# weleen/AGRL.pytorch

Measured on AMD Instinct MI355X. Metric: frames/sec (fwd+GCN+distmat), MARS seq_len=8, higher is better.
Workload: dtype fp16; 1 GPU; MARS seq_len=8 bs=32/GPU fp16 fwd+distmat (BASELINE configs[1]): 256x128 frames, VMGN ResNet50x2-branch + 2 graph layers, cosine distmat vs resident 12180 x 4096 gallery; global_batch=32, seq_len=8, gallery_rows_per_gpu=12180, parallelism=dp1, hip_graph=False, ranks=1, devices_visible=1, library=libagrl_hip.so, clip_batches_rotated=3, clip_bytes_rotated=301989888

## Files before the change

agrl.pytorch_amd/torchreid/_hip.py:

```python
from __future__ import annotations

import ctypes as C
import os
import threading

import torch

F32 = 0
LP16 = 1
F32X3 = 2
F32H3P = 4
F32H3 = 3
FRAMES_NCHW = 0
FRAMES_NHWC = 1
METRIC_EUCLIDEAN = 0
METRIC_COSINE = 1

LP_NAME = os.environ.get("AGRL_HIP_LP16")
if LP_NAME is None:
    LP_NAME = os.environ.get("AGRL_HIP_PRECISION") if os.environ.get("AGRL_HIP_PRECISION") in ("fp16", "bf16") else "fp16"
if LP_NAME not in ("fp16", "bf16"):
    raise ValueError("AGRL_HIP_LP16 must be fp16 or bf16, not %r" % LP_NAME)
LP_DTYPE = torch.float16 if LP_NAME == "fp16" else torch.bfloat16

_HERE = os.path.dirname(os.path.abspath(__file__))
LIB_PATH = os.environ.get(
    "AGRL_HIP_LIB", os.path.normpath(os.path.join(_HERE, "..", "lib", "libagrl_hip.so" if LP_NAME == "fp16" else "libagrl_hip_bf16.so"))
)


class HipLibraryError(RuntimeError):
    """libagrl_hip.so is missing or incomplete."""


class HipKernelError(RuntimeError):
    """An entry point of libagrl_hip.so returned a non-zero status."""


_p = C.c_void_p
_i = C.c_int
_f = C.c_float

SIGNATURES = {
    "agrl_stem_conv_bn_relu_maxpool": [_p, _p, _p, _p, _i, _i, _i, _i, _p],
    "agrl_stem_conv_bn_relu_maxpool_lp16": [_p, _p, _p, _p, _i, _i, _i, _p],
    "agrl_conv2d_bn_act": [_p, _p, _p, _p, _p, _i, _i, _i, _i, _i, _i, _i, _i, _i, _i, _i, _p],
    "agrl_conv1x1_dual_split16": [_p, _p, _p, _p, _p] + [_i] * 8 + [_f, _i, _i, _p],
    "agrl_stem_split16": [_p, _p, _p, _p, _p, _i, _i, _i, _f, _p],
    "agrl_stem_conv_bn_relu_maxpool_u8": [_p, _p, _i, _p, _p, _p, _i, _i, _i, _i, _p],
    "agrl_stem_conv_bn_relu_maxpool_lp16_u8": [_p, _p, _i, _p, _p, _p, _i, _i, _i, _p],
    "agrl_stem_split16_u8": [_p, _p, _i, _p, _p, _p, _p, _i, _i, _i, _f, _p],
    "agrl_frames_normalize_u8": [_p, _p, _i, _p, _i, _i, _i, _p],
    "agrl_split16_planes": [_p, _p, C.c_longlong, _i, _i, _p],
    "agrl_split16_weight_planes": [_p, _p, C.c_longlong, _i, _f, _p],
    "agrl_split16_weights_inloop": [_p, _p, C.c_longlong, _i, _p],
    "agrl_conv1x1_split16": [_p, _p, _p, _p, _p, _i, _i, _i, _i, _f, _i, _p],
    "agrl_conv1x1_split16_dual": [_p, _p, _p, _p, _p, _i, _i, _i, _i, _i, _f, _i, _p],
    "agrl_conv1x1_split16_pool": [_p, _p, _p, _p, _p, _i, _i, _i, _i, _i, _i, C.POINTER(_i), _i, _i, _f, _i, _p],
    "agrl_conv3x3_packed_split16": [_p, _p, _p, _p, _i, _i, _i, _i, _i, _i, _f, _p],
    "agrl_conv2d_bn_act_split16": [_p, _p, _p, _p, _p] + [_i] * 10 + [_f, _i, _i, _p],
    "agrl_bottleneck_tail": [_p, _p, _p, _p, _p, _p, _p, _p, _p, _p, _p, _i, _i, _i, _i, _i, _p],
    "agrl_bottleneck_seam_packed_bytes": [_i, _i, _i],
    "agrl_bottleneck_seam_pack": [_p, _p, _p, _i, _i, _i, _p],
    "agrl_bottleneck_seam": [_p, _p, _p, _p, _p, _p, _p, _i, _i, _i, _i, _p],
    "agrl_conv3x3_packed_bytes": [_i, _i],
    "agrl_conv1x1_packed_bytes": [_i, _i],
    "agrl_conv1x1_pack": [_p, _p, _i, _i, _p],
    "agrl_conv1x1_packed_bn_act": [_p, _p, _p, _p, _p, _i, _i, _i, _i, _i, _p],
    "agrl_conv1x1_packed_res_bn_act": [_p, _p, _p, _p, _p, _i, _i, _i, _i, _p],
    "agrl_conv1x1_packed_res_pool": [_p, _p, _p, _p, _p, _p, _i, _i, _i, _i, _i, _i, C.POINTER(_i), _i, _i, _p],
    "agrl_conv1x1_packed_dual_duo": [_p, _p, _p, _p, _p, _i, _i, _i, _i, _i, _p],
    "agrl_conv1x1_packed_dual_strided": [_p, _p, _p, _p, _p, _i, _i, _i, _i, _i, _i, _i, _i, _p],
    "agrl_conv3x3_pack": [_p, _p, _i, _i, _p],
    "agrl_conv3x3_packed_bn_act": [_p, _p, _p, _p, _i, _i, _i, _i, _i, _i, _p],
    "agrl_bottleneck_block": [_p, _p, _p, _p, _p, _p, _p, _p, _p, _p, _p, _p, _p, _i, _i, _i, _i, _i, _i, _p],
    "agrl_conv1x1_dual_bn_act": [_p, _p, _p, _p, _p, _i, _i, _i, _i, _i, _p],
    "agrl_conv1x1_bn_act_pool": [_p, _p, _p, _p, _p, _p, _p, _i, _i, _i, _i, _i, _i, C.POINTER(_i), _i, _i, _p],
    "agrl_linear_nobias": [_p, _p, _p, _i, _i, _i, _i, _p],
    "agrl_part_pool": [_p, _p, _p, _p, _p, _i, _i, _i, _i, C.POINTER(_i), _i, _i, _p],
    "agrl_clip_pool": [_p, _p, _i, _i, _i, _i, _p],
    "agrl_graph_gram": [_p, _p, _i, _i, _i, _i, _p],
    "agrl_graph_pair_product": [_p, _p, _p, _p, _i, _i, _i, _p],
    "agrl_graph_finalize": [_p, _i, _p, _p, _i, _i, _i, _i, _i, _p],
    "agrl_graph_propagate": [_p, _p, _p, _p, _p, _f, _f, _f, _p, _p, _i, _i, _i, _p],
    "agrl_pam_pool": [_p, _p, _p, _p, _i, _i, _i, _i, _i, C.POINTER(_i), _i, _i, _p],
    "agrl_pam_combine": [_p, _p, _p, _f, _p, _p, _i, _i, _p],
    "agrl_graph_apply": [_p, _p, _p, _i, _i, _i, _i, _p],
    "agrl_graph_tracklet_operand": [_p, _p, _i, _p, _p, _i, _i, _i, _i, _i, _i, _i, _p],
    "agrl_graph_finalize_bits": [_p, _i, _p, _p, _i, _i, _i, _i, _i, _p],
    "agrl_pose_adjacency_bits": [_p, _p, _p, _i, _i, _i, _i, C.c_float, C.c_float, _p],
    "agrl_adjacency_pack": [_p, _p, _i, _i, _p],
    "agrl_graph_linear_mix": [_p, _p, _p, _p, _p, _f, _f, _f, _p, _i, _i, _i, _i, _p],
    "agrl_row_sqnorm": [_p, _p, _i, _i, _i, _p],
    "agrl_attn_pool_bnneck": [_p, _p, _p, _p, _p, _p, _p, _p, _p, _p, _i, _i, _i, _i, _i, _p],
    "agrl_attn_tail": [_p, _p, _p, _p, _p, _p, _p, _p, _p, _p, _p, _p, _p, _i, _i, _i, _i, _i, _p],
    "agrl_row_l2_normalize": [_p, _p, _i, _i, _i, _i, _i, _p],
    "agrl_distmat_split16": [_p, _p, _p, _p, _p, _i, _i, _i, _i, _i, _f, _p, C.c_size_t, _p],
    "agrl_distmat": [_p, _p, _p, _p, _p, _i, _i, _i, _i, _i, _i, _p, C.c_size_t, _p],
    "agrl_pose_adjacency": [_p, _p, _p, _i, _i, _i, _i, C.c_float, C.c_float, _p],
    "agrl_re_ranking_workspace": [_i, _i, _i],
    "agrl_re_ranking": [_p, _p, _p, _i, _i, _i, _i, C.c_double, _p, _i, _p, C.c_size_t, _p],
    "agrl_rank_topk": [_p, _i, _i, _i, _i, _i, _p, _p, _p],
    "agrl_distmat_topk_workspace": [_i, _i],
    "agrl_distmat_topk": [_p, _p, _p, _p, _i, _i, _i, _i, _i, _i, _i, _p, _p, _p, C.c_size_t, _p, C.c_size_t, _p],
    "agrl_rank_argsort": [_p, _i, _i, _i, _p, _p],
    "agrl_rank_mars": [_p, _p, _p, _p, _p, _i, _i, _i, _p, _p, _p],
    "agrl_rank_market1501": [_p, _i, _i, _i, _p, _p, _p, _p, _i, _p, _p, _p, _p],
    "agrl_triplet_hard_mine": [_p, _p, _i, _i, _p, _p, _p, _p, _p],
    "agrl_axpby": [_p, _p, _f, _f, _p, C.c_size_t, _p],
    "agrl_part_pool_backward": [_p, _p, _p, _p, _i, _i, _i, _i, _i, C.POINTER(_i), _i, _p],
    "agrl_attn_pool_backward": [_p, _p, _p, _i, _i, _i, _i, _p],
    "agrl_graph_matrix_backward": [_p, _i, _p, _p, _i, _i, _i, _i, _p],
    "agrl_xent_label_smooth": [_p, _p, _i, _i, _f, _p, _p, _p, _p],
    "agrl_triplet_loss": [_p, _p, _i, _i, _f, _i, _p, _p, _p, _p, _p, _p, _p, _p],
    "agrl_bn_workspace": [_i, _i],
    "agrl_bn_stats": [_p, _p, _p, _i, _i, _p, C.c_size_t, _p],
    "agrl_conv2d_stats": [_p, _p, _p, _p, C.c_size_t] + [_i] * 10 + [_p],
    "agrl_bn_stats_from_partials": [_p, _i, _i, _i, _p, _p, _p, C.c_size_t, _p],
    "agrl_bn_fold_train": [_p, _p, _p, _p, _f, _f, C.c_longlong, _p, _p, _p, _p, _p, _p, _i, _p],
    "agrl_bn_apply": [_p, _p, _p, _p, _p, _p, _i, _i, _i, _f, _p],
    "agrl_bn_backward": [_p, _p, _p, _p, _p, _p, _p, _i, _f, _p, _p, _p, _p, _i, _i, _p, C.c_size_t, _p],
    "agrl_im2col_t": [_p, _p, _i, _i, _i, _i, _i, _i, _i, _i, _i, _p],
    "agrl_gemm_nt_splitk": [_p, _p, _p, _i, _i, _i, _i, _p, C.c_size_t, _p],
    "agrl_im2col_rows": [_p, _p] + [_i] * 10 + [_p],
    "agrl_conv_wgrad_workspace": [_i] * 9,
    "agrl_conv_wgrad_plan": [_i] * 10 + [C.POINTER(_i)],
    "agrl_conv_wgrad": [_p, _p, _p] + [_i] * 10 + [_p, C.c_size_t, _p],
    "agrl_maxpool3x3s2": [_p, _p, _p, _i, _i, _i, _i, _p],
    "agrl_maxpool3x3s2_backward": [_p, _p, _p, _i, _i, _i, _i, _p],
    "agrl_diag_read_stream": [_p, C.c_size_t, _p, _i, _p],
    "agrl_optim_geometry": [C.POINTER(_i), C.POINTER(_i), C.POINTER(_i)],
    "agrl_adam_step": [_p, _i, _p, _i] + [_f] * 7 + [_i, _i, _p],
    "agrl_sgd_step": [_p, _i, _p, _i, _f, _f, _f, _i, _i, _i, _i, _p],
}

_lock = threading.Lock()
_lib = None


def lib():
    global _lib
    if _lib is not None:
        return _lib
    with _lock:
        if _lib is not None:
            return _lib
        if not os.path.exists(LIB_PATH):
            raise HipLibraryError(
                "libagrl_hip.so not found at %s -- build it with `python __graft_entry__.py` "
                "(or `make -C agrl.pytorch_amd/csrc`); the HIP path has no fallback" % LIB_PATH
            )
        try:
            h = C.CDLL(LIB_PATH)
        except OSError as e:
            raise HipLibraryError("cannot load %s: %s" % (LIB_PATH, e))
        for name, argtypes in SIGNATURES.items():
            try:
                fn = getattr(h, name)
            except AttributeError:
                raise HipLibraryError("%s does not export %s" % (LIB_PATH, name))
            fn.argtypes = argtypes
            fn.restype = _i
        h.agrl_re_ranking_workspace.restype = C.c_size_t
        h.agrl_bn_workspace.restype = C.c_size_t
        h.agrl_conv_wgrad_workspace.restype = C.c_size_t
        h.agrl_distmat_topk_workspace.restype = C.c_size_t
        h.agrl_bottleneck_seam_packed_bytes.restype = C.c_longlong
        h.agrl_conv3x3_packed_bytes.restype = C.c_longlong
        h.agrl_conv1x1_packed_bytes.restype = C.c_longlong
        for name in ("agrl_reload_options", "agrl_built_with_ablation", "agrl_lp16_is_f16"):
            getattr(h, name).argtypes = []
            getattr(h, name).restype = _i
        h.agrl_version.restype = _i
        h.agrl_last_error.restype = C.c_char_p
        if bool(h.agrl_lp16_is_f16()) != (LP_NAME == "fp16"):
            raise HipLibraryError("%s stores 16-bit data as %s but AGRL_HIP_LP16 asks for %s" % (
                LIB_PATH, "fp16" if h.agrl_lp16_is_f16() else "bf16", LP_NAME))
        _lib = h
    return _lib


RELOAD_HOOKS = []


def reload_options():
    lib().agrl_reload_options()
    for hook in RELOAD_HOOKS:
        hook()


def available() -> bool:
    try:
        lib()
        return True
    except HipLibraryError:
        return False


def _check(name, status):
    if status != 0:
        msg = lib().agrl_last_error()
        raise HipKernelError("%s failed (%d): %s" % (name, status, msg.decode() if msg else "?"))


def stream_ptr(device=None):
    return torch.cuda.current_stream(device).cuda_stream


def ptr(t):
    if t is None:
        return None
    assert t.is_cuda, "HIP entry points take device tensors"
    assert t.is_contiguous(), "HIP entry points take contiguous tensors"
    return t.data_ptr()


def dtype_code(dt):
    if dt == torch.float32:
        return F32
    if dt == LP_DTYPE:
        return LP16
    raise TypeError("unsupported dtype %s (float32 / %s only: the loaded library's 16-bit type is %s)" % (dt, LP_DTYPE, LP_NAME))


PROFILE = None
PROFILE_TAG = None


def call(name, *args):
    fn = getattr(lib(), name)
    if PROFILE is None:
        _check(name, fn(*args))
        return
    stream = torch.cuda.ExternalStream(args[-1]) if args[-1] else torch.cuda.current_stream()
    start, end = torch.cuda.Event(enable_timing=True), torch.cuda.Event(enable_timing=True)
    start.record(stream)
    _check(name, fn(*args))
    end.record(stream)
    global PROFILE_TAG
    PROFILE.append((name, start, end, PROFILE_TAG))
    PROFILE_TAG = None
```

agrl.pytorch_amd/torchreid/hip_ops.py:

```python
from __future__ import annotations

import ctypes as C
import os

import torch

from . import _hip
from ._hip import F32, LP16, LP_DTYPE, LP_NAME, METRIC_COSINE, METRIC_EUCLIDEAN, call, dtype_code, ptr


import contextlib
import threading
import weakref

_MODE = threading.local()


@contextlib.contextmanager
def f32_split(on=True):
    prev = getattr(_MODE, 'split', False)
    _MODE.split = bool(on)
    try:
        yield
    finally:
# ... 458 lines not shown


def bottleneck_seam(y2, packed, b3, residual, b1_next, dims):
    Cmid, Cout, Cnext = dims
    N, H, W, C = y2.shape
    M = N * H * W
    assert y2.dtype == LP_DTYPE and C == Cmid and residual.shape == (N, H, W, Cout) and residual.dtype == y2.dtype and M % 128 == 0
    assert y2.is_contiguous() and residual.is_contiguous()
    out = torch.empty((N, H, W, Cout), dtype=y2.dtype, device=y2.device)
    z = torch.empty((N, H, W, Cnext), dtype=y2.dtype, device=y2.device)
    if _hip.PROFILE is not None:
        _hip.PROFILE_TAG = {"flops": 2.0 * M * (Cmid * Cout + Cout * Cnext),
                            "bytes": 2.0 * (y2.numel() + residual.numel() + out.numel() + z.numel()) + packed.numel(),
                            "conv": (1, 1, Cmid, Cout, H, W)}
    with _dev(y2):
        call("agrl_bottleneck_seam", ptr(y2), ptr(packed), ptr(b3), ptr(residual), ptr(out), ptr(b1_next), ptr(z), M, Cmid, Cout,
             Cnext, _stream(y2))
    return out, z


def conv3x3_packed_enabled():
    return True


def conv3x3_packed_supported(w_ohwi, H=None, W=None):
    return (w_ohwi.dtype == LP_DTYPE and w_ohwi.dim() == 4 and tuple(w_ohwi.shape[1:3]) == (3, 3) and w_ohwi.shape[3] % 64 == 0
            and w_ohwi.shape[3] >= 128 and (w_ohwi.shape[0] % 256 == 0 or w_ohwi.shape[0] == 128) and (H is None or (H % 16 == 0 and W % 8 == 0)))


def conv3x3_pack(w_ohwi):
    assert conv3x3_packed_supported(w_ohwi)
    Cout, Cin = w_ohwi.shape[0], w_ohwi.shape[3]
    if Cout == 128:
        w_ohwi = torch.cat([w_ohwi, torch.zeros_like(w_ohwi)], dim=0)
        Cout = 256
    w_ohwi = w_ohwi.contiguous()
    nbytes = int(_hip.lib().agrl_conv3x3_packed_bytes(Cin, Cout))
    assert nbytes == 2 * w_ohwi.numel()
    packed = torch.empty((nbytes,), dtype=torch.uint8, device=w_ohwi.device)
    with _dev(w_ohwi):
        call("agrl_conv3x3_pack", ptr(w_ohwi), ptr(packed), Cin, Cout, _stream(w_ohwi))
    return packed


def conv3x3_packed(x, packed, bias, Cout, relu=True):
    N, H, W, Cin = x.shape
    assert x.dtype == LP_DTYPE and x.is_contiguous() and packed.numel() == 2 * 9 * Cin * max(Cout, 256)
    out = torch.empty((N, H, W, Cout), dtype=x.dtype, device=x.device)
    if _hip.PROFILE is not None:
        _hip.PROFILE_TAG = {"flops": 2.0 * N * H * W * 9 * Cin * Cout, "bytes": 2.0 * (x.numel() + out.numel()) + 2.0 * 9 * Cin * Cout,
                            "conv": (3, 1, Cin, Cout, H, W)}
    with _dev(x):
        call("agrl_conv3x3_packed_bn_act", ptr(x), ptr(packed), ptr(bias), ptr(out), N, H, W, Cin, Cout, 1 if relu else 0, _stream(x))
    return out


def conv1x1_packed_supported(w):
    w2 = w.reshape(w.shape[0], -1) if w.dim() == 4 and tuple(w.shape[1:3]) == (1, 1) else w
    return w2.dtype == LP_DTYPE and w2.dim() == 2 and w2.shape[1] % 128 == 0 and w2.shape[0] % 256 == 0


def conv1x1_pack(w):
    assert conv1x1_packed_supported(w)
    w = w.reshape(w.shape[0], -1).contiguous()
    Cout, K = w.shape
    nbytes = int(_hip.lib().agrl_conv1x1_packed_bytes(K, Cout))
    assert nbytes == 2 * w.numel()
    packed = torch.empty((nbytes,), dtype=torch.uint8, device=w.device)
    with _dev(w):
        call("agrl_conv1x1_pack", ptr(w), ptr(packed), K, Cout, _stream(w))
    return packed


def conv1x1_packed(x, packed, bias, Cout, relu=True, x2=None, duo=False):
    N, H, W, K1 = x.shape
    K2 = 0 if x2 is None else x2.shape[3]
    M = N * H * W
    assert x.dtype == LP_DTYPE and x.is_contiguous() and packed.numel() == 2 * (K1 + K2) * Cout
    assert x2 is None or (x2.dtype == x.dtype and x2.is_contiguous() and tuple(x2.shape[:3]) == (N, H, W))
    out = torch.empty((N, H, W, Cout), dtype=x.dtype, device=x.device)
    if _hip.PROFILE is not None:
        _hip.PROFILE_TAG = {"flops": 2.0 * M * (K1 + K2) * Cout,
                            "bytes": 2.0 * (x.numel() + (0 if x2 is None else x2.numel()) + out.numel()) + packed.numel(),
                            "conv": (1, 1, K1 + K2, Cout, H, W)}
    with _dev(x):
        if duo and x2 is not None:
            call("agrl_conv1x1_packed_dual_duo", ptr(x), ptr(x2), ptr(packed), ptr(bias), ptr(out), M, K1, K2, Cout, 1 if relu else 0, _stream(x))
        else:
            call("agrl_conv1x1_packed_bn_act", ptr(x), ptr(x2), ptr(packed), ptr(bias), ptr(out), M, K1, K2, Cout, 1 if relu else 0, _stream(x))
    return out


def conv1x1_packed_dual_strided(x, x2, packed, bias, Cout, stride, relu=True):
    N, Hi, Wi, K1 = x.shape
    Ho, Wo = (Hi - 1) // stride + 1, (Wi - 1) // stride + 1
    K2 = x2.shape[3]
    assert x.dtype == LP_DTYPE and x2.dtype == LP_DTYPE and x.is_contiguous() and x2.is_contiguous()
    assert tuple(x2.shape[:3]) == (N, Ho, Wo) and packed.numel() == 2 * (K1 + K2) * Cout
    out = torch.empty((N, Ho, Wo, Cout), dtype=x.dtype, device=x.device)
    M = N * Ho * Wo
    if _hip.PROFILE is not None:
        _hip.PROFILE_TAG = {"flops": 2.0 * M * (K1 + K2) * Cout, "bytes": 2.0 * (M * K1 + x2.numel() + out.numel()) + packed.numel(),
                            "conv": (1, 1, K1 + K2, Cout, Ho, Wo)}
    with _dev(x):
        call("agrl_conv1x1_packed_dual_strided", ptr(x), ptr(x2), ptr(packed), ptr(bias), ptr(out), N, Hi, Wi, stride, K1, K2, Cout,
             1 if relu else 0, _stream(x))
# ... 812 lines not shown
```

agrl.pytorch_amd/torchreid/models/_vmgn_hip.py:

```python
from __future__ import annotations

import os

import torch

from torchreid import hip_ops as ops
from torchreid import _hip

_PRECISIONS = {'fp32': torch.float32, ops.LP_NAME: ops.LP_DTYPE, 'bf16x3': torch.float32, 'fp16x3': torch.float32}


def _fold_conv_bn(conv, bn, dtype, split16=False):
    w = conv.weight.detach().float()
    scale = bn.weight.detach().float() / torch.sqrt(bn.running_var.detach().float() + bn.eps)
    shift = bn.bias.detach().float() - bn.running_mean.detach().float() * scale
    w = (w * scale.view(-1, 1, 1, 1)).permute(0, 2, 3, 1).contiguous()
    if split16:
        assert dtype == torch.float32
        return ops.split16_inloop_weights(w), shift.contiguous()
    return w.to(dtype).contiguous(), shift.contiguous()


def check_packed_range(pack, where="vmgn"):
    def walk(obj, path):
# ... 5 lines not shown
            for k, v in obj.items():
                walk(v, "%s.%s" % (path, k))
        elif isinstance(obj, (list, tuple)):
            for i, v in enumerate(obj):
                walk(v, "%s[%d]" % (path, i))
    walk({k: v for k, v in pack.items() if k != 'fingerprint'}, "pack")


def _fold_bn1d(bn):
    scale = bn.weight.detach().float() / torch.sqrt(bn.running_var.detach().float() + bn.eps)
    shift = bn.bias.detach().float() - bn.running_mean.detach().float() * scale
    return scale.contiguous(), shift.contiguous()


def _pack_stage(stage, dtype, seam=False, split16=False):
    blocks = []
    for unit in stage:
        blk = {
            'c1': _fold_conv_bn(unit.conv1, unit.bn1, dtype, split16),
            'c2': _fold_conv_bn(unit.conv2, unit.bn2, dtype, split16),
            'c3': _fold_conv_bn(unit.conv3, unit.bn3, dtype, split16),
            'stride': unit.conv2.stride[0],
            'ds': None,
        }
        if unit.downsample is not None:
            blk['ds'] = _fold_conv_bn(unit.downsample[0], unit.downsample[1], dtype, split16)
            blk['ds_stride'] = unit.downsample[0].stride[0]
            if split16 and blk['ds_stride'] == blk['stride'] and blk['ds'][0].shape[3] % 32 == 0 and blk['c3'][0].shape[3] % 32 == 0:
                cout = blk['c3'][0].shape[0]
                wd = ops.split16_true_weights(blk['ds'][0])
                w3 = ops.split16_true_weights(blk['c3'][0])
                blk['dual16'] = (ops.split16_inloop_weights(torch.cat([wd.view(cout, -1), w3.view(cout, -1)], dim=1).contiguous()),
                                 (blk['ds'][1] + blk['c3'][1]).contiguous())
            if dtype == ops.LP_DTYPE and blk['ds_stride'] == 1 and blk['stride'] == 1:
                cout = blk['c3'][0].shape[0]
                blk['dual'] = (torch.cat([blk['ds'][0].view(cout, -1), blk['c3'][0].view(cout, -1)], dim=1).contiguous(),
                               (blk['ds'][1] + blk['c3'][1]).contiguous())
                if (ops.conv1x1_packed_supported(blk['dual'][0]) and blk['dual'][0].shape[1] >= 1536
                        and blk['ds'][0].shape[3] % 128 == 0 and blk['c3'][0].shape[3] % 128 == 0):
                    blk['dualp'] = ops.conv1x1_pack(blk['dual'][0])
            if dtype == ops.LP_DTYPE and blk['ds_stride'] > 1 and blk['ds_stride'] == blk['stride']:
                cout = blk['c3'][0].shape[0]
                dual_w = torch.cat([blk['ds'][0].view(cout, -1), blk['c3'][0].view(cout, -1)], dim=1).contiguous()
                if (ops.conv1x1_packed_supported(dual_w) and blk['ds'][0].shape[3] % 128 == 0 and blk['c3'][0].shape[3] % 128 == 0):
                    blk['dualps'] = ops.conv1x1_pack(dual_w)
                    blk['dualps_bias'] = (blk['ds'][1] + blk['c3'][1]).contiguous()
        if dtype == ops.LP_DTYPE and ops.conv1x1_packed_supported(blk['c1'][0]) and blk['c1'][0].shape[3] >= 1024:
            blk['c1p'] = ops.conv1x1_pack(blk['c1'][0])
        if (dtype == ops.LP_DTYPE and blk['ds'] is None and ops.conv1x1_packed_supported(blk['c3'][0])
                and blk['c3'][0].shape[0] >= 2048):
            blk['c3p'] = ops.conv1x1_pack(blk['c3'][0])
        if dtype == ops.LP_DTYPE and blk['stride'] == 1 and ops.conv3x3_packed_supported(blk['c2'][0]):
            blk['c2p'] = ops.conv3x3_pack(blk['c2'][0])
        blocks.append(blk)
    if seam and dtype == ops.LP_DTYPE:
        for blk, nxt in zip(blocks[:-1], blocks[1:]):
            if ops.bottleneck_seam_supported(blk['c3'][0], nxt['c1'][0]):
                blk['seam'] = ops.bottleneck_seam_pack(blk['c3'][0], nxt['c1'][0])
                blk['seam_dims'] = (blk['c3'][0].shape[3], blk['c3'][0].shape[0], nxt['c1'][0].shape[0])
    return blocks


def K_OK(w):
    return w.dim() == 2 and w.shape[1] % 32 == 0


def _fingerprint(model):
    return tuple((t.data_ptr(), t._version) for t in list(model.parameters()) + list(model.buffers()))


def pack_weights(model, device, precision):
    ops.check_precision(precision)
    key = (device.index if device.index is not None else torch.cuda.current_device(), precision)
    cached = model._hip_packs.get(key)
    if cached is not None and (model.hip_static_weights or cached['fingerprint'] == _fingerprint(model)):
        return cached
    first = next(model.parameters())
    if first.device != device:
        raise RuntimeError('model parameters live on {} but the input is on {}'.format(first.device, device))
    dtype = _PRECISIONS[precision]
    s16 = precision == 'fp16x3'
    with torch.no_grad():
        stem_w, stem_b = _fold_conv_bn(model.conv1, model.bn1, torch.float32)
        pack = {
            'dtype': dtype,
            'stem': (stem_w, stem_b),
            'stem_lp': ops.pack_stem_weights_lp16(stem_w) if dtype == ops.LP_DTYPE else None,
            'stem_s16': ops.pack_stem_weights_split16(stem_w) if s16 else None,
            'trunk': _pack_stage(model.layer1, dtype, split16=s16) + _pack_stage(model.layer2, dtype, split16=s16) + _pack_stage(model.layer3, dtype, seam=True, split16=s16),
            'graph': [],
        }
        if hasattr(model, 'layer4_1'):
            pack['l4_1'] = _pack_stage(model.layer4_1, dtype, split16=s16)
            pack['l4_2'] = _pack_stage(model.layer4_2, dtype, split16=s16)
            pack['g_bn'] = _fold_bn1d(model.global_bottleneck)
            pack['a_bn'] = _fold_bn1d(model.att_bottleneck)
        else:
            pack['l4'] = _pack_stage(model.layer4, dtype, split16=s16)
            pack['a_bn'] = _fold_bn1d(model.bottleneck)
            pack['g_bn'] = (torch.ones_like(pack['a_bn'][0]), torch.zeros_like(pack['a_bn'][1]))
        for layer in model.graph_layers:
            scale, shift = _fold_bn1d(layer.bn)
            gw = layer.linear.weight.detach().to(dtype).contiguous()
            if s16 and K_OK(gw):
                gw = ops.split16_inloop_weights(gw)
                scale = (scale * gw.agrl_unscale).contiguous()
# ... 24 lines not shown
        check_packed_range(pack)
    pack['fingerprint'] = _fingerprint(model)
    model._hip_packs[key] = pack
    return pack


def _pack_planes(blk):
    def true_w(pair):
        return ops.split16_true_weights(pair[0])

    w1, w2, w3 = true_w(blk['c1']), true_w(blk['c2']), true_w(blk['c3'])
    K1, K3c, mid, cout = w1.shape[3], w3.shape[3], w1.shape[0], w3.shape[0]
    if blk['stride'] != 1 or mid % 256 or cout % 256 or K1 % 128 or K3c % 128 or tuple(w2.shape[1:3]) != (3, 3) or w2.shape[3] % 64:
        return False
    p3 = {}
    t, u = ops.split16_plane_weights(w1.view(mid, K1), pair_first=True)
    p3['c1'] = (ops.conv1x1_pack(t), u, blk['c1'][1], mid)
    t, u = ops.split16_plane_weights(w2)
    p3['c2'] = (ops.conv3x3_pack(t), u, blk['c2'][1], w2.shape[0])
    if blk['ds'] is not None:
        if blk['ds_stride'] != 1:
            return False
        wd = true_w(blk['ds'])
        Kd = wd.shape[3]
        if Kd % 128:
            return False
        t, u = ops.split16_plane_weights(torch.cat([wd.view(cout, Kd), w3.view(cout, K3c)], dim=1), segments=[Kd, K3c], pair_first=True)
        p3['dual'] = (ops.conv1x1_pack(t), u, (blk['ds'][1] + blk['c3'][1]).contiguous(), cout)
    else:
        t, u = ops.split16_plane_weights(w3.view(cout, K3c))
        p3['c3'] = (ops.conv1x1_pack(t), u, blk['c3'][1], cout)
    blk['p3'] = p3
    return True


def _run_block_planes(x3, blk, pool=None):
    p3 = blk['p3']
    xp, rop = 1, 2
    y = ops.conv1x1_split16(x3, p3['c1'][0], p3['c1'][1], p3['c1'][2], p3['c1'][3], layout=xp)
    y = ops.conv3x3_split16(y, p3['c2'][0], p3['c2'][1], p3['c2'][2], p3['c2'][3])
    if 'dual' in p3:
        assert pool is None
        d = p3['dual']
        return ops.conv1x1_split16(x3, d[0], d[1], d[2], d[3], x2=y, layout=xp | rop)
    c = p3['c3']
    if pool is not None:
        return ops.conv1x1_split16_pool(y, c[0], c[1], c[2], c[3], x3, pool[0], pool[1], layout=rop)
    return ops.conv1x1_split16(y, c[0], c[1], c[2], c[3], residual3=x3, layout=rop)


def _conv2(y, blk):
    if 'c2p' in blk and y.shape[1] % 16 == 0 and y.shape[2] % 8 == 0:
        return ops.conv3x3_packed(y, blk['c2p'], blk['c2'][1], blk['c2'][0].shape[0], True)
    return ops.conv_bn_act(y, blk['c2'][0], blk['c2'][1], blk['stride'], 1, True)


def _conv1(x, blk):
    if 'c1p' in blk and x.is_contiguous():
        return ops.conv1x1_packed_res(x, blk['c1p'], blk['c1'][1], blk['c1'][0].shape[0], None, True)
    return ops.conv_bn_act(x, blk['c1'][0], blk['c1'][1], 1, 0, True)


def _run_block_inloop(x, blk, out_planes=0):
    y = ops.conv_bn_act(x, blk['c1'][0], blk['c1'][1], 1, 0, True, out_presplit=True)
    y = ops.conv_bn_act(y, blk['c2'][0], blk['c2'][1], blk['stride'], 1, True, x_presplit=True, out_presplit=True)
    if 'dual16' in blk and x.is_contiguous():
        return ops.conv1x1_dual_split16(x, y, blk['dual16'][0], blk['dual16'][1], blk['stride'], True, x2_presplit=True, out_planes=out_planes)
    shortcut = x if blk['ds'] is None else ops.conv_bn_act(x, blk['ds'][0], blk['ds'][1], blk['ds_stride'], 0, False)
    out = ops.conv_bn_act(y, blk['c3'][0], blk['c3'][1], 1, 0, True, residual=shortcut, x_presplit=True)
    return ops.to_split16_planes(out, out_planes) if out_planes else out


def _is_inloop(blk):
    return getattr(blk['c1'][0], 'agrl_presplit', False)


def _run_trunk(a, blocks):
    z = None
    for i, blk in enumerate(blocks):
        if _is_inloop(blk):
            a = _run_block_inloop(a, blk)
            continue
        nxt = blocks[i + 1] if i + 1 < len(blocks) else None
        y = z if z is not None else ops.conv_bn_act(a, blk['c1'][0], blk['c1'][1], 1, 0, True)
        if nxt is not None:
            ds = None if blk['ds'] is None else (blk['ds'][0], blk['ds_stride'])
            if ops.bottleneck_block_supported(y, blk['c2'][0], blk['stride'], blk['c3'][0], nxt['c1'][0], ds) and (
                    ds is None or a.shape[3] == 64):
                if ds is None:
                    a, z = ops.bottleneck_block(y, blk['c2'][0], blk['c2'][1], blk['c3'][0], blk['c3'][1], a,
                                                nxt['c1'][0], nxt['c1'][1])
                else:
                    a, z = ops.bottleneck_block(y, blk['c2'][0], blk['c2'][1], blk['c3'][0], blk['c3'][1], None,
                                                nxt['c1'][0], nxt['c1'][1], shortcut=(a, blk['ds'][0], blk['ds'][1]))
                continue
        y = _conv2(y, blk)
        fusable = nxt is not None and ops.bottleneck_tail_supported(y, blk['c3'][0], nxt['c1'][0])
        if fusable and blk['ds'] is not None and ops.bottleneck_tail_supported(
                y, blk['c3'][0], nxt['c1'][0], (blk['ds'][0], blk['ds_stride'])) and a.shape[3] == 64:
            a, z = ops.bottleneck_tail(y, blk['c3'][0], blk['c3'][1], None, nxt['c1'][0], nxt['c1'][1],
                                       shortcut=(a, blk['ds'][0], blk['ds'][1]))
            continue
        if ('dualps' in blk and a.is_contiguous() and y.is_contiguous() and a.dtype == y.dtype and a.shape[0] == y.shape[0]
                and tuple(y.shape[1:3]) == tuple((d - 1) // blk['stride'] + 1 for d in a.shape[1:3])):
            a = ops.conv1x1_packed_dual_strided(a, y, blk['dualps'], blk['dualps_bias'], blk['c3'][0].shape[0], blk['stride'], True)
            z = None
# ... 202 lines not shown
```

include/agrl_hip.h:

```cpp
#ifndef AGRL_HIP_H
#define AGRL_HIP_H

#include <stddef.h>
#include <stdint.h>

#ifdef __cplusplus
extern "C" {
#endif

#define AGRL_F32 0
#define AGRL_LP16 1
#define AGRL_BF16 AGRL_LP16
#define AGRL_F32X3 2
#define AGRL_F32H3 3
#define AGRL_F32H3P 4

#define AGRL_METRIC_EUCLIDEAN 0
#define AGRL_METRIC_COSINE 1

typedef void* agrl_stream_t;

int agrl_version(void);
const char* agrl_last_error(void);

// ... 24 lines not shown
int agrl_frames_normalize_u8(const unsigned char* x, const float* table, int layout, float* out, int N, int H, int W,
                             agrl_stream_t stream);

int agrl_conv2d_bn_act(const void* x, const void* w, const float* bias, const void* residual,
                       void* out, int N, int H, int W, int Cin, int Cout, int R, int S, int stride,
                       int pad, int relu, int dtype, agrl_stream_t stream);

int agrl_conv2d_bn_act_split16(const void* x, const void* w_scaled, const float* bias, const void* residual, void* out, int N,
                               int H, int W, int Cin, int Cout, int R, int S, int stride, int pad, int relu, float w_unscale,
                               int x_presplit, int out_presplit, agrl_stream_t stream);

int agrl_split16_weights_inloop(const float* w_scaled, void* out, long long rows, int K, agrl_stream_t stream);

int agrl_conv1x1_dual_split16(const void* x, const void* x2, const void* w_scaled, const float* bias, void* out, int N, int H, int W,
                              int stride, int K1, int K2, int Cout, int relu, float w_unscale, int x2_presplit, int out_planes,
                              agrl_stream_t stream);

int agrl_split16_planes(const float* x, void* out, long long rows, int C, int nplanes, agrl_stream_t stream);
int agrl_split16_weight_planes(const float* x, void* out, long long rows, int C, float scale, agrl_stream_t stream);
int agrl_conv1x1_split16(const void* x, const void* packed, const float* bias, const void* residual, void* out, int M, int K3,
                         int Cout, int relu, float w_unscale, int layout, agrl_stream_t stream);
int agrl_conv1x1_split16_dual(const void* x, const void* x2, const void* packed, const float* bias, void* out, int M, int K1_3,
                              int K2_3, int Cout, int relu, float w_unscale, int layout, agrl_stream_t stream);
int agrl_conv1x1_split16_pool(const void* x, const void* packed, const float* bias, const void* residual, float* pool_out, int N,
                              int H, int W, int K3, int Cout, int relu, const int* splits, int n_splits, int mean, float w_unscale,
                              int layout, agrl_stream_t stream);
int agrl_conv3x3_packed_split16(const void* x, const void* packed, const float* bias, void* out, int N, int H, int W, int Cin3,
                                int Cout, int relu, float w_unscale, agrl_stream_t stream);

int agrl_conv1x1_dual_bn_act(const void* x1, const void* x2, const void* w, const float* bias, void* out, int M,
                             int K1, int K2, int Cout, int relu, agrl_stream_t stream);

int agrl_conv1x1_bn_act_pool(const void* x, const void* w, const float* bias, const void* residual,
                             void* out, float* pool_out, void* pool_out_lp, int N, int H, int W,
                             int Cin, int Cout, int relu, const int* splits, int n_splits, int mean,
                             agrl_stream_t stream);

int agrl_bottleneck_tail(const void* y2, const void* w3, const float* b3, const void* residual,
                         const void* x_short, const void* w_short, const float* b_short, void* out,
                         const void* w1_next, const float* b1_next, void* z, int M, int Cmid, int Cout,
                         int Cnext, int Cshort, agrl_stream_t stream);

long long agrl_bottleneck_seam_packed_bytes(int Cmid, int Cout, int Cnext);
int agrl_bottleneck_seam_pack(const void* w3, const void* w1_next, void* packed, int Cmid, int Cout, int Cnext,
                              agrl_stream_t stream);
int agrl_bottleneck_seam(const void* y2, const void* packed, const float* b3, const void* residual, void* out,
                         const float* b1_next, void* z, int M, int Cmid, int Cout, int Cnext, agrl_stream_t stream);

long long agrl_conv3x3_packed_bytes(int Cin, int Cout);
int agrl_conv3x3_pack(const void* w_ohwi, void* packed, int Cin, int Cout, agrl_stream_t stream);
int agrl_conv3x3_packed_bn_act(const void* x, const void* packed, const float* bias, void* out, int N, int H, int W, int Cin,
                               int Cout, int relu, agrl_stream_t stream);

long long agrl_conv1x1_packed_bytes(int K, int Cout);
int agrl_conv1x1_pack(const void* w, void* packed, int K, int Cout, agrl_stream_t stream);
int agrl_conv1x1_packed_bn_act(const void* x, const void* x2, const void* packed, const float* bias, void* out, int M, int K1,
                               int K2, int Cout, int relu, agrl_stream_t stream);

int agrl_conv1x1_packed_res_bn_act(const void* x, const void* packed, const float* bias, const void* residual, void* out, int M,
                                   int K, int Cout, int relu, agrl_stream_t stream);
int agrl_conv1x1_packed_res_pool(const void* x, const void* packed, const float* bias, const void* residual, float* pool_out,
                                 void* pool_out_lp, int N, int H, int W, int K, int Cout, int relu, const int* splits,
                                 int n_splits, int mean, agrl_stream_t stream);
int agrl_conv1x1_packed_dual_duo(const void* x, const void* x2, const void* packed, const float* bias, void* out, int M, int K1,
                                 int K2, int Cout, int relu, agrl_stream_t stream);
int agrl_conv1x1_packed_dual_strided(const void* x, const void* x2, const void* packed, const float* bias, void* out, int N, int Hi,
                                     int Wi, int stride, int K1, int K2, int Cout, int relu, agrl_stream_t stream);

int agrl_bottleneck_block(const void* z, const void* w2, const float* b2, const void* w3, const float* b3,
                          const void* residual, const void* x_short, const void* w_short, const float* b_short,
                          void* out, const void* w1_next, const float* b1_next, void* z_next, int F, int H, int W,
                          int Cmid, int Cout, int Cnext, agrl_stream_t stream);

int agrl_linear_nobias(const void* x, const void* w, float* y, int M, int K, int Nout,
                       int in_dtype, agrl_stream_t stream);


int agrl_pose_adjacency(const float* poses, const unsigned char* detected, float* adj, int B, int S,
                        int num_split, int pyramid_part, float height, float threshold, agrl_stream_t stream);
int agrl_pose_adjacency_bits(const float* poses, const unsigned char* detected, uint32_t* adj_bits, int B, int S, int num_split,
                             int pyramid_part, float height, float threshold, agrl_stream_t stream);
int agrl_adjacency_pack(const float* adj, uint32_t* adj_bits, int B, int V, agrl_stream_t stream);


int agrl_part_pool(const void* x4_1, const void* x4_2, float* gsum, float* nodes, void* nodes_lp,
                   int F, int h, int w, int C, const int* splits, int n_splits, int dtype,
                   agrl_stream_t stream);


int agrl_graph_gram(const float* f, float* gram_part, int B, int V, int C, int cslice,
                    agrl_stream_t stream);

int agrl_graph_finalize(const float* gram_part, int nz, const float* adj, float* G, int B, int V,
                        int use_pose, int learn_graph, int mask_diag, agrl_stream_t stream);
int agrl_graph_finalize_bits(const float* gram_part, int nz, const uint32_t* adj_bits, float* G, int B, int V, int use_pose,
                             int learn_graph, int mask_diag, agrl_stream_t stream);

int agrl_graph_apply(const float* G, const float* f, void* out, int out_dtype, int B, int V, int C, agrl_stream_t stream);
int agrl_graph_tracklet_operand(const float* f, const void* adj, int adj_packed, float* G_out, void* out, int out_dtype, int B,
                                int V, int C, int use_pose, int learn_graph, int mask_diag, agrl_stream_t stream);
int agrl_graph_linear_mix(const void* p_op, const void* w, const float* f, const float* bn_scale, const float* bn_shift,
                          float keep, float gamma, float slope, float* out, int M, int K, int Nout, int in_dtype,
                          agrl_stream_t stream);

int agrl_graph_propagate(const float* f, const float* h, const float* G, const float* bn_scale,
                         const float* bn_shift, float keep, float gamma, float slope, float* out, void* out_lp,
// ... 138 lines not shown
```

Baseline: 72130 frames/s.

## Add packed, pipelined stride-2 3x3 conv kernel for bottleneck downsampling blocks

```diff
diff --git a/agrl.pytorch_amd/csrc/conv3x3_s2.hip b/agrl.pytorch_amd/csrc/conv3x3_s2.hip
--- /dev/null
+++ b/agrl.pytorch_amd/csrc/conv3x3_s2.hip
@@ -0,0 +1,244 @@
+#include "fat_dev.h"
+
+namespace {
+
+struct S2Params {
+    const unsigned char* x;
+    const unsigned char* wpk;
+    const float* bias;
+    unsigned char* out;
+    int H, W, OH, OW, Cin, Cout, relu;
+};
+
+constexpr int S2_RING = 12;
+constexpr int S2_FPS = 9 * 2;
+constexpr int S2_BODY = 2 * S2_FPS;
+constexpr int S2_PIECES = 36, S2_PPW = 9;
+constexpr int S2_SLAB = S2_PIECES * 1024;
+constexpr int S2_PIXELS = 33 * 17;
+static_assert(S2_BODY % S2_RING == 0 && S2_PPW <= S2_FPS && S2_PIECES == 4 * S2_PPW, "ring turns per body; one patch piece per fragment; no dummy pieces");
+static_assert(S2_RING <= S2_FPS && S2_FPS - S2_RING <= S2_PPW, "the prologue replays the tail of ONE slab");
+
+__device__ __host__ constexpr int s2_plane_w(int pl) { return (pl & 1) ? 8 : 9; }
+__device__ __host__ constexpr int s2_plane_base(int pl) { return pl == 0 ? 0 : pl == 1 ? 17 * 9 : pl == 2 ? 17 * 17 : 17 * 17 + 16 * 9; }
+__device__ inline int s2_g(int row, int col) { return ((col >> 2) & 1) ^ ((row & 1) << 1); }
+
+struct S2Sched {
+    int allowed[S2_BODY];
+};
+constexpr S2Sched make_s2_sched() {
+    S2Sched s{};
+    int issued[4][S2_BODY] = {};
+    int seq = 0;
+    for (int p = S2_BODY - S2_RING; p < S2_BODY; ++p) {
+        issued[0][p + S2_RING - S2_BODY] = seq++;
+        if (p % S2_FPS < S2_PPW) seq += 1;
+    }
+    for (int k = 0; k < 3; ++k)
+        for (int p = 0; p < S2_BODY; ++p) {
+            if (k == 1) s.allowed[p] = seq - 1 - issued[k][p];
+            const int q = p + S2_RING;
+            if (q >= S2_BODY) issued[k + 1][q - S2_BODY] = seq++;
+            else issued[k][q] = seq++;
+            if (p % S2_FPS < S2_PPW) seq += 1;
+        }
+    return s;
+}
+struct S2SchedOf {
+    static constexpr S2Sched value = make_s2_sched();
+};
+constexpr int S2_PIECE_WAIT = S2_FPS - S2_PPW;
+
+__global__ __launch_bounds__(256, 2) void conv3x3_s2_kernel(const S2Params p) {
+    using SCHED = S2SchedOf;
+    using std::integral_constant;
+    constexpr int NBF = 8;
+    __shared__ __attribute__((aligned(16))) unsigned char smem_[2 * S2_SLAB];
+    lds_u8_t* const smem = (lds_u8_t*)smem_;
+    const unsigned lds0 = (unsigned)(size_t)smem;
+
+    const int tid = threadIdx.x;
+    const int lane = tid & 63;
+    const int wave = __builtin_amdgcn_readfirstlane(tid >> 6);
+    const unsigned lane16 = (unsigned)lane * 16u;
+    const int frow = lane & 15, fchunk = lane >> 4;
+
+    const int nNt = p.Cout >> 7;
+    int bid = blockIdx.x;
+    {
+        const int nblk = gridDim.x, q = nblk >> 3, r = nblk & 7;
+        const int xcd = bid & 7, within = bid >> 3;
+        bid = (xcd < r ? xcd * (q + 1) : r * (q + 1) + (xcd - r) * q) + within;
+    }
+    const int mt = bid / nNt, nt = bid - mt * nNt;
+    const int tw = p.OW >> 3, th = p.OH >> 4;
+    const int img = mt / (tw * th);
+    const int trem = mt - img * (tw * th);
+    const int oy0 = (trem / tw) << 4, ox0 = (trem % tw) << 3;
+
+    unsigned poff[S2_PPW];
+    bool pok[S2_PPW];
+    const unsigned char* zsrc = reinterpret_cast<const unsigned char*>(&g_zero16);
+#pragma unroll
+    for (int i = 0; i < S2_PPW; ++i) {
+        const int q = (wave + 4 * i) * 16 + (lane >> 2);
+        const int pl = q < s2_plane_base(1) ? 0 : q < s2_plane_base(2) ? 1 : q < s2_plane_base(3) ? 2 : 3;
+        const int qq = q - s2_plane_base(pl);
+        const int pw = s2_plane_w(pl);
+        const int row = qq / pw, col = qq - row * pw;
+        const int iy = 2 * oy0 - 1 + 2 * row + (pl >> 1), ix = 2 * ox0 - 1 + 2 * col + (pl & 1);
+        pok[i] = q < S2_PIXELS && (unsigned)iy < (unsigned)p.H && (unsigned)ix < (unsigned)p.W;
+        poff[i] = (unsigned)((((size_t)img * p.H + iy) * p.W + ix) * p.Cin * 2 + (((lane & 3) ^ s2_g(row, col)) << 4));
+    }
+    auto stage_patch_piece = [&](int slab, int buf, int i) {
+        const unsigned dst = lds0 + buf * S2_SLAB + (wave + 4 * i) * 1024;
+        fat_dma(pok[i] ? p.x + poff[i] + slab * 64 : zsrc, __builtin_amdgcn_readfirstlane(dst));
+    };
+
+    const int fp = frag_px(frow);
+    const int r0 = fp >> 3, x0 = fp & 7;
+    int tbase[9];
+#pragma unroll
+    for (int t = 0; t < 9; ++t) {
+        const int tr = t / 3, ts = t % 3, pl = (tr & 1) * 2 + (ts & 1);
+        const int row = r0 + (tr >> 1), col = x0 + (ts >> 1);
+        tbase[t] = (s2_plane_base(pl) + row * s2_plane_w(pl) + col) * 64 + ((fchunk ^ s2_g(row, col)) << 4);
+    }
+
+    const int nbody = p.Cin >> 6;
+    const unsigned char* wstream = p.wpk + (size_t)(nt * 4 + wave) * nbody * (S2_BODY * 1024);
+    u32x4_t wr[S2_RING];
+    auto issue_w = [&](auto slot_c, const unsigned char* body_base, auto pos_c) {
+        constexpr int SLOT = decltype(slot_c)::value, POS = decltype(pos_c)::value;
+        fat_gload<(POS & 3) * 1024>(wr[SLOT], lane16, body_base + (POS & ~3) * 1024);
+    };
+
+    asm volatile("" ::: "a63");
+    sfor<2 * NBF>([&](auto qc) { fat_zero<decltype(qc)::value>(); });
+
+    sfor<S2_FPS - S2_RING>([&](auto ic) { stage_patch_piece(0, 0, decltype(ic)::value); });
+    sfor<S2_RING>([&](auto ic) {
+        constexpr int I = decltype(ic)::value, POS = S2_FPS - S2_RING + I;
+        issue_w(ic, wstream, ic);
+        if constexpr (POS < S2_PPW) stage_patch_piece(0, 0, POS);
+    });
+
+    u32x4_t xf[NBF];
+    for (int it = 0; it < nbody; ++it) {
+        const bool more = it + 1 < nbody;
+        const unsigned char* ws = wstream + (size_t)it * (S2_BODY * 1024);
+        const unsigned char* wsn = wstream + (size_t)(more ? it + 1 : 0) * (S2_BODY * 1024);
+        sfor<S2_BODY>([&](auto pc) {
+            constexpr int P = decltype(pc)::value;
+            constexpr int HALF = P / S2_FPS, PS = P % S2_FPS, TAP = PS >> 1, A = PS & 1, SL = P % S2_RING;
+            const lds_u8_t* sp = smem + HALF * S2_SLAB;
+            auto ldx = [&](auto tap_c, auto b_c) {
+                constexpr int T = decltype(tap_c)::value, B = decltype(b_c)::value;
+                return *reinterpret_cast<const lds_u32x4_t*>(sp + tbase[T] + B * (2 * 64 * s2_plane_w(T % 3)));
+            };
+            if constexpr (PS == 0) {
+                asm volatile("s_waitcnt vmcnt(%0)" ::"n"(S2_PIECE_WAIT) : "memory");
+                __builtin_amdgcn_s_barrier();
+                asm volatile("" ::: "memory");
+                sfor<NBF>([&](auto bc) { xf[decltype(bc)::value] = ldx(integral_constant<int, 0>{}, bc); });
+            }
+            fat_wait<SCHED::value.allowed[P]>(wr[SL]);
+            sfor<NBF>([&](auto bc) {
+                constexpr int B = decltype(bc)::value;
+                fat_mfma<A * NBF + B>(wr[SL], xf[B]);
+                if constexpr (A == 1 && TAP + 1 < 9) {
+                    __builtin_amdgcn_sched_barrier(0);
+                    xf[B] = ldx(integral_constant<int, TAP + 1>{}, bc);
+                }
+            });
+            __builtin_amdgcn_sched_barrier(0);
+            constexpr int Q = P + S2_RING;
+            if constexpr (Q >= S2_BODY) issue_w(integral_constant<int, SL>{}, wsn, integral_constant<int, Q - S2_BODY>{});
+            else issue_w(integral_constant<int, SL>{}, ws, integral_constant<int, Q>{});
+            if constexpr (PS < S2_PPW) stage_patch_piece(HALF == 0 ? 2 * it + 1 : (more ? 2 * it + 2 : 2 * it + 1), HALF ^ 1, PS);
+        });
+    }
+#pragma unroll
+    for (int i = 0; i < S2_RING; ++i) asm volatile("" : "+v"(wr[i]));
+    asm volatile("s_waitcnt vmcnt(0)" ::: "memory");
+#pragma unroll
+    for (int i = 0; i < S2_RING; ++i) asm volatile("" : "+v"(wr[i]));
+    asm volatile("s_nop 15\n\ts_nop 15" ::: "memory");
+
+    const int cb = nt * 128 + wave * 32 + 8 * fchunk;
+    const float4 b0 = *reinterpret_cast<const float4*>(p.bias + cb);
+    const float4 b1 = *reinterpret_cast<const float4*>(p.bias + cb + 4);
+    sfor<NBF>([&](auto bc) {
+        constexpr int B = decltype(bc)::value;
+        const f32x4_t lo = fat_read<B>(), hi = fat_read<NBF + B>();
+        float v[8] = {lo[0] + b0.x, lo[1] + b0.y, lo[2] + b0.z, lo[3] + b0.w, hi[0] + b1.x, hi[1] + b1.y, hi[2] + b1.z, hi[3] + b1.w};
+        if (p.relu) {
+#pragma unroll
+            for (int e = 0; e < 8; ++e) v[e] = relu_nan(v[e]);
+        }
+        const int m = B * 16 + fp;
+        const size_t gm = ((size_t)img * p.OH + oy0 + (m >> 3)) * p.OW + ox0 + (m & 7);
+        *reinterpret_cast<uint4*>(p.out + (gm * p.Cout + cb) * 2) =
+            make_uint4(pack_lp16x2(v[0], v[1]), pack_lp16x2(v[2], v[3]), pack_lp16x2(v[4], v[5]), pack_lp16x2(v[6], v[7]));
+    });
+}
+
+__global__ void conv3x3_s2_pack_kernel(const lp16_t* __restrict__ w, uint4* __restrict__ wpk, int Cin, int Cout) {
+    const int nslab = Cin >> 5;
+    const long long total = (long long)(Cout >> 7) * 4 * nslab * S2_FPS * 64;
+    for (long long t = blockIdx.x * (long long)blockDim.x + threadIdx.x; t < total; t += (long long)gridDim.x * blockDim.x) {
+        const int lane = (int)(t & 63);
+        long long r = t >> 6;
+        const int q = (int)(r % S2_FPS);
+        r /= S2_FPS;
+        const int slab = (int)(r % nslab);
+        r /= nslab;
+        const int wv = (int)(r & 3), nt = (int)(r >> 2);
+        const int a = q & 1, tap = q >> 1;
+        const int i = lane & 15, f = lane >> 4;
+        const int ch = nt * 128 + wv * 32 + 8 * (i >> 2) + 4 * a + (i & 3);
+        wpk[t] = *reinterpret_cast<const uint4*>(w + ((size_t)ch * 9 + tap) * Cin + slab * 32 + f * 8);
+    }
+}
+
+bool s2_channels_ok(int Cin, int Cout) { return Cin % 64 == 0 && Cin >= 128 && (Cout == 128 || (Cout > 0 && Cout % 256 == 0)); }
+
+}
+
+extern "C" long long agrl_conv3x3_s2_packed_bytes(int Cin, int Cout) {
+    if (!s2_channels_ok(Cin, Cout)) return 0;
+    return (long long)Cout * 9 * Cin * 2;
+}
+
+extern "C" int agrl_conv3x3_s2_pack(const void* w_ohwi, void* packed, int Cin, int Cout, agrl_stream_t stream) {
+    AGRL_CHECK_ARG(w_ohwi && packed, "agrl_conv3x3_s2_pack: null pointer");
+    AGRL_CHECK_ARG(s2_channels_ok(Cin, Cout), "agrl_conv3x3_s2_pack: needs Cin %% 64 == 0 (>= 128) and Cout == 128 or Cout %% 256 == 0, got %d / %d", Cin, Cout);
+    AGRL_CHECK_ARG((((uintptr_t)w_ohwi | (uintptr_t)packed) & 15) == 0, "agrl_conv3x3_s2_pack: pointers must be 16-byte aligned");
+    hipLaunchKernelGGL(conv3x3_s2_pack_kernel, dim3(512), dim3(256), 0, (hipStream_t)stream, reinterpret_cast<const lp16_t*>(w_ohwi),
+                       reinterpret_cast<uint4*>(packed), Cin, Cout);
+    AGRL_CHECK_LAUNCH("agrl_conv3x3_s2_pack");
+    return 0;
+}
+
+extern "C" int agrl_conv3x3_s2_packed_bn_act(const void* x, const void* packed, const float* bias, void* out, int N, int H, int W, int Cin,
+                                             int Cout, int relu, agrl_stream_t stream) {
+    AGRL_CHECK_ARG(x && packed && bias && out, "agrl_conv3x3_s2_packed_bn_act: null pointer");
+    const int OH = H > 0 ? (H - 1) / 2 + 1 : 0, OW = W > 0 ? (W - 1) / 2 + 1 : 0;
+    AGRL_CHECK_ARG(N > 0 && H > 0 && W > 0 && OH % 16 == 0 && OW % 8 == 0 && s2_channels_ok(Cin, Cout),
+                   "agrl_conv3x3_s2_packed_bn_act: needs output maps made of whole 16 x 8 blocks, Cin %% 64 == 0 (>= 128), Cout == 128 or Cout %% 256 == 0; got %dx%d -> %dx%d, %d->%d",
+                   H, W, OH, OW, Cin, Cout);
+    AGRL_CHECK_ARG((size_t)N * H * W * (size_t)Cin * 2 < (1ull << 32) && (size_t)N * OH * OW * (size_t)Cout * 2 < (1ull << 32),
+                   "agrl_conv3x3_s2_packed_bn_act: maps beyond 4 GB are not addressed");
+    AGRL_CHECK_ARG((((uintptr_t)x | (uintptr_t)packed | (uintptr_t)bias | (uintptr_t)out) & 15) == 0, "agrl_conv3x3_s2_packed_bn_act: pointers must be 16-byte aligned");
+    S2Params p;
+    p.x = reinterpret_cast<const unsigned char*>(x);
+    p.wpk = reinterpret_cast<const unsigned char*>(packed);
+    p.bias = bias;
+    p.out = reinterpret_cast<unsigned char*>(out);
+    p.H = H; p.W = W; p.OH = OH; p.OW = OW; p.Cin = Cin; p.Cout = Cout; p.relu = relu;
+    const long long nwg = (long long)N * (OH >> 4) * (OW >> 3) * (Cout >> 7);
+    AGRL_CHECK_ARG(nwg < (1ll << 31), "agrl_conv3x3_s2_packed_bn_act: too many workgroups");
+    hipLaunchKernelGGL(conv3x3_s2_kernel, dim3((unsigned)nwg), dim3(256), 0, (hipStream_t)stream, p);
+    AGRL_CHECK_LAUNCH("agrl_conv3x3_s2_packed_bn_act");
+    return 0;
+}
diff --git a/agrl.pytorch_amd/torchreid/_hip.py b/agrl.pytorch_amd/torchreid/_hip.py
--- a/agrl.pytorch_amd/torchreid/_hip.py
+++ b/agrl.pytorch_amd/torchreid/_hip.py
@@ -73,6 +73,9 @@
     "agrl_conv1x1_packed_dual_strided": [_p, _p, _p, _p, _p, _i, _i, _i, _i, _i, _i, _i, _i, _p],
     "agrl_conv3x3_pack": [_p, _p, _i, _i, _p],
     "agrl_conv3x3_packed_bn_act": [_p, _p, _p, _p, _i, _i, _i, _i, _i, _i, _p],
+    "agrl_conv3x3_s2_packed_bytes": [_i, _i],
+    "agrl_conv3x3_s2_pack": [_p, _p, _i, _i, _p],
+    "agrl_conv3x3_s2_packed_bn_act": [_p, _p, _p, _p, _i, _i, _i, _i, _i, _i, _p],
     "agrl_bottleneck_block": [_p, _p, _p, _p, _p, _p, _p, _p, _p, _p, _p, _p, _p, _i, _i, _i, _i, _i, _i, _p],
     "agrl_conv1x1_dual_bn_act": [_p, _p, _p, _p, _p, _i, _i, _i, _i, _i, _p],
     "agrl_conv1x1_bn_act_pool": [_p, _p, _p, _p, _p, _p, _p, _i, _i, _i, _i, _i, _i, C.POINTER(_i), _i, _i, _p],
@@ -167,6 +170,7 @@
         h.agrl_distmat_topk_workspace.restype = C.c_size_t
         h.agrl_bottleneck_seam_packed_bytes.restype = C.c_longlong
         h.agrl_conv3x3_packed_bytes.restype = C.c_longlong
+        h.agrl_conv3x3_s2_packed_bytes.restype = C.c_longlong
         h.agrl_conv1x1_packed_bytes.restype = C.c_longlong
         for name in ("agrl_reload_options", "agrl_built_with_ablation", "agrl_lp16_is_f16"):
             getattr(h, name).argtypes = []
@@ -227,7 +231,7 @@
 PROFILE_TAG = None
 
 
-def call(name, *args):
+def call(name, *args, profile_name=None):
     fn = getattr(lib(), name)
     if PROFILE is None:
         _check(name, fn(*args))
@@ -238,5 +242,5 @@
     _check(name, fn(*args))
     end.record(stream)
     global PROFILE_TAG
-    PROFILE.append((name, start, end, PROFILE_TAG))
+    PROFILE.append((profile_name or name, start, end, PROFILE_TAG))
     PROFILE_TAG = None
diff --git a/agrl.pytorch_amd/torchreid/hip_ops.py b/agrl.pytorch_amd/torchreid/hip_ops.py
--- a/agrl.pytorch_amd/torchreid/hip_ops.py
+++ b/agrl.pytorch_amd/torchreid/hip_ops.py
@@ -534,6 +534,38 @@
                             "conv": (3, 1, Cin, Cout, H, W)}
     with _dev(x):
         call("agrl_conv3x3_packed_bn_act", ptr(x), ptr(packed), ptr(bias), ptr(out), N, H, W, Cin, Cout, 1 if relu else 0, _stream(x))
+    return out
+
+
+def conv3x3_s2_supported(w_ohwi, H=None, W=None):
+    return (w_ohwi.dtype == LP_DTYPE and w_ohwi.dim() == 4 and tuple(w_ohwi.shape[1:3]) == (3, 3) and w_ohwi.shape[3] % 64 == 0
+            and w_ohwi.shape[3] >= 128 and (w_ohwi.shape[0] % 256 == 0 or w_ohwi.shape[0] == 128)
+            and (H is None or (H > 0 and W > 0 and ((H - 1) // 2 + 1) % 16 == 0 and ((W - 1) // 2 + 1) % 8 == 0)))
+
+
+def conv3x3_s2_pack(w_ohwi):
+    assert conv3x3_s2_supported(w_ohwi)
+    Cout, Cin = w_ohwi.shape[0], w_ohwi.shape[3]
+    w_ohwi = w_ohwi.contiguous()
+    nbytes = int(_hip.lib().agrl_conv3x3_s2_packed_bytes(Cin, Cout))
+    assert nbytes == 2 * w_ohwi.numel()
+    packed = torch.empty((nbytes,), dtype=torch.uint8, device=w_ohwi.device)
+    with _dev(w_ohwi):
+        call("agrl_conv3x3_s2_pack", ptr(w_ohwi), ptr(packed), Cin, Cout, _stream(w_ohwi))
+    return packed
+
+
+def conv3x3_s2_packed(x, packed, bias, Cout, relu=True):
+    N, H, W, Cin = x.shape
+    assert x.dtype == LP_DTYPE and x.is_contiguous() and packed.numel() == 2 * 9 * Cin * Cout
+    OH, OW = (H - 1) // 2 + 1, (W - 1) // 2 + 1
+    out = torch.empty((N, OH, OW, Cout), dtype=x.dtype, device=x.device)
+    if _hip.PROFILE is not None:
+        _hip.PROFILE_TAG = {"flops": 2.0 * N * OH * OW * Cout * 9 * Cin, "bytes": 2.0 * (x.numel() + 9 * Cin * Cout + out.numel()),
+                            "conv": (3, 2, Cin, Cout, OH, OW)}
+    with _dev(x):
+        call("agrl_conv3x3_s2_packed_bn_act", ptr(x), ptr(packed), ptr(bias), ptr(out), N, H, W, Cin, Cout, 1 if relu else 0, _stream(x),
+             profile_name="agrl_conv2d_bn_act")
     return out
 
 
diff --git a/agrl.pytorch_amd/torchreid/models/_vmgn_hip.py b/agrl.pytorch_amd/torchreid/models/_vmgn_hip.py
--- a/agrl.pytorch_amd/torchreid/models/_vmgn_hip.py
+++ b/agrl.pytorch_amd/torchreid/models/_vmgn_hip.py
@@ -81,6 +81,8 @@
             blk['c3p'] = ops.conv1x1_pack(blk['c3'][0])
         if dtype == ops.LP_DTYPE and blk['stride'] == 1 and ops.conv3x3_packed_supported(blk['c2'][0]):
             blk['c2p'] = ops.conv3x3_pack(blk['c2'][0])
+        if dtype == ops.LP_DTYPE and blk['stride'] == 2 and ops.conv3x3_s2_supported(blk['c2'][0]):
+            blk['c2s2'] = ops.conv3x3_s2_pack(blk['c2'][0])
         blocks.append(blk)
     if seam and dtype == ops.LP_DTYPE:
         for blk, nxt in zip(blocks[:-1], blocks[1:]):
@@ -211,6 +213,9 @@
 def _conv2(y, blk):
     if 'c2p' in blk and y.shape[1] % 16 == 0 and y.shape[2] % 8 == 0:
         return ops.conv3x3_packed(y, blk['c2p'], blk['c2'][1], blk['c2'][0].shape[0], True)
+    if ('c2s2' in blk and y.is_contiguous() and ops.conv3x3_s2_supported(blk['c2'][0], y.shape[1], y.shape[2])
+            and ops.switch('AGRL_CONV3X3_S2') != '0'):
+        return ops.conv3x3_s2_packed(y, blk['c2s2'], blk['c2'][1], blk['c2'][0].shape[0], True)
     return ops.conv_bn_act(y, blk['c2'][0], blk['c2'][1], blk['stride'], 1, True)
 
 
diff --git a/include/agrl_hip.h b/include/agrl_hip.h
--- a/include/agrl_hip.h
+++ b/include/agrl_hip.h
@@ -100,6 +100,11 @@
 int agrl_conv3x3_packed_bn_act(const void* x, const void* packed, const float* bias, void* out, int N, int H, int W, int Cin,
                                int Cout, int relu, agrl_stream_t stream);
 
+long long agrl_conv3x3_s2_packed_bytes(int Cin, int Cout);
+int agrl_conv3x3_s2_pack(const void* w_ohwi, void* packed, int Cin, int Cout, agrl_stream_t stream);
+int agrl_conv3x3_s2_packed_bn_act(const void* x, const void* packed, const float* bias, void* out, int N, int H, int W, int Cin,
+                                  int Cout, int relu, agrl_stream_t stream);
+
 long long agrl_conv1x1_packed_bytes(int K, int Cout);
 int agrl_conv1x1_pack(const void* w, void* packed, int K, int Cout, agrl_stream_t stream);
 int agrl_conv1x1_packed_bn_act(const void* x, const void* x2, const void* packed, const float* bias, void* out, int M, int K1,
```

Result: no change. 72410 frames/s (median of 6 runs) (+0.4%).
